# kunalchelani/EdgeGaussians

Measured on AMD Instinct MI355X. Metric: train-step Gaussians*views/sec, higher is better.
Workload: dtype f32; 1 GPU; config2: 100000 Gaussians (5:1 anisotropic, scale 0.004, opacity U(0.05,0.9)), 50 views @512x512, real poses of scan 00004926 (intrinsics 800->512); synthetic wireframe edge maps, loss whole/bg_edge_ratio 4:1; n_gaussians=100000, views=50, width=512, height=512, poses=real poses of scan 00004926 (intrinsics 800->512); synthetic wireframe edge maps, largest_tile_population=2957, gaussian_row_order=morton, binning=segmented, steps_per_native_enqueue=50, forward_mode=chained (exact transmittance stop resolved inside the forward kernel), parallelism=single GPU

## Files before the change

### edgegaussians_amd/_lib.py

```python
from __future__ import annotations

import ctypes as C
import os
from typing import Optional

import torch

_HERE = os.path.dirname(os.path.abspath(__file__))
LIB_PATH = os.path.join(_HERE, "libedgegs.so")

_vp = C.c_void_p
_i32 = C.c_int32
_i64 = C.c_int64
_u32 = C.c_uint32
_f = C.c_float

FLAG_LOG_SCALES = 1
FLAG_LOGIT_OPACITIES = 2
FLAG_ANTIALIASED = 4
FLAG_TIGHT_TILES = 8
FLAG_ABSGRAD_WRITE = 16
FLAG_FRONT_PREFIX = 32
PREFIX_HERE_MAX_TILES = 2560
REWALK_SPECULATE = -2
# ... 45 lines not shown
    "eg_tile_offsets": [_vp, _i32, _i64, _vp, _vp, _vp, _vp],
    "eg_tile_emit": [_vp, _vp, _vp, _vp, _u32, _i32, _i32, _i32, _vp, _vp, _i64, _vp, _vp, _vp],
    "eg_project_bin": [_vp] * 6 + [_i32, _i32, _i32, _u32, _vp, _vp, _vp, _i64, _vp, _vp, _vp, _vp, _vp],
    "eg_sort_pairs": [_vp, _vp, _i32, _i64, _vp, _vp, _i32, _vp],
    "eg_project_emit": [_vp] * 6 + [_i32, _i32, _i32, _u32, _vp, _vp, _i32, _vp, _vp, _i32, _vp, _vp, _vp],
    "eg_sort_segments": [_vp, _vp, _i32, _i32, _vp, _vp, _vp, _vp, _vp, _vp, _i32, _i32, _vp],
    "eg_composite_fwd_segments": [_vp] * 7 + [_i32, _i32, _vp, _vp, _vp, _vp, _vp, _f, _vp, _vp, _vp, _i64, _vp, _vp, _i32, _vp],
    "eg_composite_fwd": [_vp, _vp, _i32, _vp, _vp, _i32, _i32, _vp, _vp, _vp, _vp, _vp, _f, _vp, _vp,
                         _vp, _vp, _i64, _vp, _vp, _i32, _vp],
    "eg_composite_bwd_colors": [_vp, _vp, _i32, _vp, _vp, _i32, _i32, _vp, _vp, _vp, _vp, _vp, _vp, _vp],
    "eg_project_bwd": [_vp] * 6 + [_i32, _i32, _i32, _f, _u32] + [_vp] * 9 + [_vp],
    "eg_absgrad_accum": [_vp, _i32, _vp, _vp],
    "eg_composite_bwd_footprint": [_vp, _i32, _i32, _i32, _vp, _vp, _vp],
    "eg_backward_fused": [_vp] * 6 + [_i32, _i32, _i32, _f, _u32] + [_vp] * 10 + [C.POINTER(AdamHyper), _vp],
    "eg_adam_multi": [_vp] * 10 + [_i32, AdamHyper, _vp, _vp, _vp],
    "eg_adam_tensor": [_vp] * 4 + [_i64, C.c_double, C.c_double, C.c_double, C.c_double, _i32, _i32, _vp],
    "eg_adam_emit": [_vp] * 10 + [_i32, AdamHyper, _vp, _vp, _vp, _vp, _i32, _i32, _u32, _vp, _vp, _i32, _vp, _vp, _i32,
                     _vp, _vp, _vp],
    "eg_project_bwd_adam": [_vp] * 6 + [_i32, _i32, _i32, _f, _u32] + [_vp] * 5 + [AdamHyper, _vp],
    "eg_mask_scan": [_vp, _i32, _vp, _vp, _vp],
    "eg_compact_rows": [_vp, _vp, _vp, _i32, _i32, _vp, _vp],
    "eg_append_rows": [_vp, _vp, _vp, _i32, _i32, _i32, _i32, _vp, _f, _vp, _vp],
    "eg_ratio_wmap": [_vp, _f, _i32, _vp, _i32, _i32, _vp, _vp],
    "eg_ratio_wmap_seeded": [_vp, _f, _i32, _i32, _i32, C.c_uint64, _i32, _vp, _vp],
    "eg_ratio_wmaps_seeded": [_i32, C.POINTER(_vp), _f, C.POINTER(_i32), C.POINTER(_i32), C.POINTER(_i32), C.POINTER(C.c_uint64),
                              _i32, _vp, _vp],
    "eg_project_hits": [_vp, _i32, _vp, _i32, _vp, _i32, _i32, _vp, _vp],
    "eg_project_visibility": [_vp, _i32, _vp, _i32, _vp, _i32, _i32, _vp, _vp],
    "eg_knn": [_vp, _i32, _i32, C.POINTER(_f), _f, C.POINTER(_i32), _vp, _vp, _vp, _vp, _vp, _vp, _vp],
    "eg_knn_small": [_vp, _i32, _i32, _vp, _vp, _vp],
    "eg_knn_auto": [_vp, _i32, _i32, _vp, _vp, _vp, _vp, _vp, _vp, _vp, _vp, _f, _vp],
    "eg_nn_query_small": [_vp, _i64, _vp, _i64, _vp, _vp, _vp],
    "eg_nn_query_auto": [_vp, _i64, _vp, _i64] + [_vp] * 8 + [_vp],
    "eg_edge_sample_count": [_vp, _i32, _vp, _i32, C.c_double, _i64, _vp, _vp, _vp, _vp, _vp],
    "eg_edge_sample_emit": [_vp, _i32, _vp, _i32, _vp, _vp, _vp, _i64, _i32, _vp, _vp, _vp, _vp],
    "eg_edge_sample": [_vp, _i32, _vp, _i32, C.c_double, _i64, _i32] + [_vp] * 7 + [C.POINTER(_i32), _vp],
    "eg_direction_loss": [_vp, _vp, _vp, _vp, _i32, _i32, _i32, _vp, _vp, _vp, _vp],
    "eg_ratio_loss": [_vp, _i32, _vp, _vp, _vp],
    "eg_regulariser_step": [_i32] + [_vp] * 7 + [_i32, _vp, _i32, _i32, _i32, _i32, _vp, _f, _f, _vp, AdamHyper, _vp],
    "eg_regulariser_step_fixed": [_i32] + [_vp] * 7 + [_i32, _vp, _i32, _i32, _i32, _i32, _vp, _f, _f, _vp, AdamHyper, _vp, _vp],
    "eg_train_step": [C.POINTER(StepArgs), _vp],
    "eg_train_steps": [C.POINTER(StepArgs), _i32, C.POINTER(_i32), C.POINTER(_vp), _vp, _vp, _vp, _vp],
    "eg_train_steps_multi": [_i32, C.POINTER(C.POINTER(StepArgs)), _i32, C.POINTER(C.POINTER(_i32)), C.POINTER(C.POINTER(_vp)),
                             C.POINTER(_vp), C.POINTER(_vp), C.POINTER(_vp), C.POINTER(_vp), _i32],
    "eg_operator_fwd": [C.POINTER(OperatorArgs), _vp],
    "eg_operator_bwd": [C.POINTER(OperatorArgs), _vp, _i64, _vp, _vp, _vp, _vp, _vp, _vp, _vp, _vp, _vp],
    "eg_train_steps_dp": [C.POINTER(StepArgs), C.POINTER(AdamHyper), _vp, _i32, C.POINTER(_i32), C.POINTER(_vp), _vp, _vp,
                          _vp, _i32, _vp],
    "eg_dp_all_reduce": [_vp, _i64, _vp],
    "eg_project_fwd_cams": [_vp] * 6 + [_i32, _i32, _i32, _i32, _f, _f, _f, _f, _u32] + [_vp] * 8 + [_vp],
    "eg_project_bwd_cams": [_vp] * 6 + [_i32, _i32, _i32, _i32, _f, _u32] + [_vp] * 7 + [_vp],
    "eg_tile_offsets_cams": [_vp, _i32, _i32, _i64, _vp, _vp, _vp, _vp],
    "eg_tile_emit_sort_cams": [_vp, _vp, _vp, _i32, _i32, _i32, _i32, _vp, _vp, C.POINTER(_i64), C.POINTER(_vp), C.POINTER(_vp),
                               C.POINTER(_vp), C.POINTER(_i32), _vp],
    "eg_composite_fwd_cams": [_i32, _vp, _i32, _vp, _i32, _i32, C.POINTER(_vp), C.POINTER(_vp), _i32, _i32, _vp, _vp, _vp,
                              C.POINTER(_vp), C.POINTER(_vp), C.POINTER(_i64), C.POINTER(_vp), _vp, _vp],
    "eg_composite_bwd_footprint_cams": [_vp, _i32, _i32, _i32, _i32, _vp, _vp, _vp],
    "eg_composite_fwd_modes_cams": [_i32, _vp, _i32, _vp, _i32, _i32, _i32, _vp, _vp, _vp, _i32, _i32, _vp, _vp, _vp, _vp],
    "eg_composite_bwd_modes_cams": [_i32, _vp, _i32, _vp, _i32, _i32, _i32, _vp, _vp, _vp, _i32, _i32, _vp, _vp, _vp, _vp,
                                    _vp, _vp, _vp, _vp],
    "eg_composite_fwd_wide_cams": [_i32, _vp, _i32, _vp, _i32, _i32, _i32, _vp, _vp, _vp, _i32, _i32, _vp, _vp, _vp, _i32, _i32,
                                   _i32, _vp],
    "eg_composite_bwd_wide_cams": [_i32, _vp, _i32, _vp, _i32, _i32, _i32, _vp, _vp, _vp, _i32, _i32, _vp, _vp, _vp, _vp,
                                   _vp, _vp, _vp, _i32, _i32, _i32, _vp],
    "eg_packed_count": [_vp] * 6 + [_i32, _i32, _i32, _i32, _f, _f, _f, _f, _u32, _vp, _vp, _vp],
    "eg_packed_write": [_vp] * 6 + [_i32, _i32, _i32, _i32, _f, _f, _f, _f, _u32, _vp, _i64] + [_vp] * 10 + [_vp],
    "eg_packed_bin": [_vp, _vp, _vp, C.POINTER(_i64), _i32, _i32, _i32, _vp, _vp, C.POINTER(_i64), _vp, _vp, _vp,
                      C.POINTER(_i32), _vp],
    "eg_packed_bwd": [_vp] * 6 + [_i32, _i32, _i32, _i32, _f, _u32, _vp, _i64] + [_vp] * 7 + [_vp],
    "eg_packed_bwd_sparse": [_vp] * 6 + [_i32, _i32, _i32, _i32, _f, _u32, _i64] + [_vp] * 8 + [_vp],
    "eg_project_bwd_viewmats": [_vp] * 6 + [_i32, _i32, _i32, _i32, _f, _u32, _vp, _vp, _i64, _vp, _vp, _vp, _vp, _vp, _i32,
                                _vp, _vp],
    "eg_sh_fwd": [_i32, _i32, _i32, _i32, _vp, _vp, _vp, _vp, _i32, _vp, _i32, _vp, _vp],
    "eg_sh_bwd": [_i32, _i32, _i32, _i32, _vp, _vp, _vp, _vp, _i32, _vp, _i32, _vp, _vp, _vp, _vp, _vp],
    "eg_train_step_batched": [C.POINTER(StepArgs), _i32, C.POINTER(_vp), C.POINTER(_vp), C.POINTER(_vp), C.POINTER(_vp), _vp],
}
EXPORTS = sorted(list(_SIGS) + ["eg_last_error_string", "eg_version", "eg_device_count",
                                 "eg_composite_workspace_bytes", "eg_composite_workspace_ctl_bytes",
                                 "eg_batched_workspace_stride", "eg_knn_auto_dims", "eg_timing_begin", "eg_timing_end",
                                 "eg_timing_stage_count", "eg_timing_stage_name", "eg_debug_fwd_profile",
                                 "eg_dp_unique_id", "eg_dp_init", "eg_dp_world", "eg_dp_shutdown", "eg_dp_host_profile", "eg_roctx_enable",
                                 "eg_dp_comm_count", "eg_dp_force_all_reduce", "eg_dp_grad_all_reduces",
                                 "eg_dp_comm_timing_begin", "eg_dp_comm_timing_end", "eg_record_xcd_shift",
                                 "eg_backward_is_fused"])

_lib: Optional[C.CDLL] = None


def load(require_device: bool = True) -> C.CDLL:
    global _lib
    if _lib is None:
        if not os.path.exists(LIB_PATH):
            raise RuntimeError(
                f"{LIB_PATH} is missing: build it with `python -m edgegaussians_amd.build` "
                "(hipcc --offload-arch=gfx950).  There is no CPU fallback in the product path.")
        lib = C.CDLL(LIB_PATH)
        for name, args in _SIGS.items():
            fn = getattr(lib, name)
            fn.argtypes = args
            fn.restype = C.c_int
        lib.eg_last_error_string.restype = C.c_char_p
        lib.eg_last_error_string.argtypes = []
        lib.eg_version.restype = C.c_int
        lib.eg_device_count.restype = C.c_int
        lib.eg_timing_begin.argtypes = [_i32]
        lib.eg_timing_end.argtypes = [C.POINTER(C.c_float), C.POINTER(_i32)]
        lib.eg_timing_stage_name.argtypes = [_i32]
        lib.eg_timing_stage_name.restype = C.c_char_p
        lib.eg_composite_workspace_bytes.restype = _i64
        lib.eg_composite_workspace_bytes.argtypes = [_i64, _i64]
        lib.eg_composite_workspace_ctl_bytes.restype = _i64
        lib.eg_composite_workspace_ctl_bytes.argtypes = [_i64, _i64]
        lib.eg_batched_workspace_stride.restype = _i64
        lib.eg_batched_workspace_stride.argtypes = [_i64, _i64]
        lib.eg_knn_auto_dims.restype = _i32
        lib.eg_knn_auto_dims.argtypes = [_i32, _i32]
        lib.eg_dp_unique_id.argtypes = [C.c_char_p, _vp]
        lib.eg_dp_init.argtypes = [C.c_char_p, _vp, _i32, _i32]
        lib.eg_dp_world.argtypes = []
        lib.eg_dp_shutdown.argtypes = []
        lib.eg_roctx_enable.argtypes = [_i32]
        lib.eg_record_xcd_shift.argtypes = [_i32]
        lib.eg_backward_is_fused.argtypes = [_i32, _i32]
        lib.eg_dp_comm_count.argtypes = []
        lib.eg_dp_force_all_reduce.argtypes = [_i32]
        lib.eg_dp_grad_all_reduces.argtypes = [C.POINTER(_i64)]
        lib.eg_dp_grad_all_reduces.restype = _i64
        lib.eg_dp_comm_timing_begin.argtypes = [_i32]
        lib.eg_dp_comm_timing_end.argtypes = [C.POINTER(C.c_float), C.POINTER(C.c_float), C.POINTER(_i32)]
        lib.eg_dp_host_profile.argtypes = [C.POINTER(C.c_double)]
        lib.eg_dp_host_profile.restype = _i64
        lib.eg_debug_fwd_profile.restype = _i64
        lib.eg_debug_fwd_profile.argtypes = [_vp, _i64]
        _lib = lib
    if require_device and not torch.cuda.is_available():
        raise RuntimeError("edgegaussians_amd needs a gfx950 GPU (torch.cuda.is_available() is False); "
                           "there is no CPU fallback in the product path")
    return _lib


def composite_workspace(max_items: int, n_tiles: int, device) -> torch.Tensor:
    lib = load()
    return torch.zeros(lib.eg_composite_workspace_bytes(max_items, n_tiles), dtype=torch.uint8, device=device)


def call(name: str, *args) -> None:
    lib = load()
    rc = getattr(lib, name)(*args)
    if rc != 0:
        raise RuntimeError(f"{name} failed (code {rc}): {lib.eg_last_error_string().decode()}")


def ptr(t: Optional[torch.Tensor]) -> Optional[int]:
    if t is None:
        return None
    assert t.is_cuda and t.is_contiguous(), "libedgegs needs contiguous device tensors"
    return t.data_ptr()


_raw_stream = getattr(torch._C, "_cuda_getCurrentRawStream", None)


def stream() -> int:
    if _raw_stream is not None:
        return _raw_stream(torch.cuda.current_device())
    return torch.cuda.current_stream().cuda_stream
```

### edgegaussians_amd/csrc/binning.hip

```cpp
#include <cstdlib>

#include "common.h"
#include "composite.h"

namespace eg {

constexpr int kBinThreads = 512;
constexpr int kMaxLdsTiles = 16384;

template <bool LDS>
__global__ void __launch_bounds__(kBinThreads)
tile_count_kernel(const float2 *__restrict__ means2d, const int *__restrict__ radii, int N, int width,
                  int height, int *__restrict__ tiles_per_gauss, int *__restrict__ tile_counts) {
  extern __shared__ __attribute__((aligned(16))) int s_hist[];
  const int tw = (width + kTile - 1) / kTile, th = (height + kTile - 1) / kTile, T = tw * th;
  if (LDS) {
    for (int t = threadIdx.x; t < T; t += kBinThreads) s_hist[t] = 0;
    __syncthreads();
  }
  const int g = blockIdx.x * kBinThreads + threadIdx.x;
  if (g < N) {
    const int radius = radii[g];
    int n = 0;
    if (radius > 0) {
// ... 149 lines not shown
      if (idx < capacity) keys[idx] = key;
    }
#undef EG_TILE_OK
}


template <int THREADS>
__device__ __forceinline__ void bitonic_lds(unsigned long long *s, int P, int k_lo, int k_hi, int tid) {
  for (int k = k_lo; k <= k_hi; k <<= 1) {
    if (k <= P) {
      const int lhk = 31 - __clz(k) - 1;
      const int mk = (1 << lhk) - 1;
      for (int i = tid; i < (P >> 1); i += THREADS) {
        const int blk = i >> lhk, off = i & mk;
        const int base = blk << (lhk + 1);
        const int lo = base + off, hi = base + k - 1 - off;
        unsigned long long a = s[lo], b = s[hi];
        if (a > b) { s[lo] = b; s[hi] = a; }
      }
      __syncthreads();
    }
    for (int j = min(k >> 2, P >> 1); j >= 1; j >>= 1) {
      const int lj = 31 - __clz(j);
      for (int i = tid; i < (P >> 1); i += THREADS) {
        const int lo = ((i >> lj) << (lj + 1)) + (i & (j - 1)), hi = lo + j;
        unsigned long long a = s[lo], b = s[hi];
        if (a > b) { s[lo] = b; s[hi] = a; }
      }
      __syncthreads();
    }
  }
}

template <int THREADS>
__device__ __forceinline__ unsigned block_reduce_u32(unsigned v, bool take_max, unsigned *wave_tmp) {
  const int tid = threadIdx.x, lane = tid & 63, wv = tid >> 6;
  constexpr int NW = THREADS / 64;
#pragma unroll
  for (int d = 32; d >= 1; d >>= 1) {
    const unsigned o = __shfl_xor(v, d, 64);
    v = take_max ? max(v, o) : min(v, o);
  }
  if (lane == 0) wave_tmp[wv] = v;
  __syncthreads();
  unsigned r = wave_tmp[0];
#pragma unroll
  for (int w = 1; w < NW; ++w) r = take_max ? max(r, wave_tmp[w]) : min(r, wave_tmp[w]);
  __syncthreads();
  return r;
}

constexpr int kMaxBucketFill = 96;
constexpr int kSortBM = 2;

struct SegTable {
  int *cursor;
  int seg_cap;
  int *tile_start, *tile_end;
  int *item_first;
  int *item_end;
  int *item_tile;
  int max_items;
  int *total;
  int4 *item_rec;
  int slice_major = 0;
  const int *item_front = nullptr;
  int middle_out = 0;
  unsigned rec_tag = 0;
  int xcd_shift = 0;
  int tw = 0;
  const float *gt = nullptr, *wmap = nullptr;
  float *loss_part = nullptr;
  int width = 0, height = 0;
  int skip_empty = 0;
  float inv_tw = 0.f;
#ifdef EG_SORT_PROF
  unsigned long long *prof = nullptr;
#endif
};
constexpr int kXcdMinTiles = 512;
constexpr int kXcdShiftDefault = 1;
constexpr int kFrontDefault = 4;

template <int THREADS, int CAP, bool LARGE, bool PREFIX3 = false>
__global__ void __launch_bounds__(THREADS, THREADS == 1024 ? 1 : 4)
tile_sort_kernel(unsigned long long *__restrict__ keys, const int *__restrict__ offsets, int T,
                 long long capacity, int small_cap, int *__restrict__ flatten_ids,
                 long long *__restrict__ isect_ids, const SegTable seg_, const Batch bt) {
  extern __shared__ __attribute__((aligned(16))) unsigned long long s[];
  SegTable seg = seg_;
  {
    const int bv = blockIdx.y;
    keys += bv * bt.keys; flatten_ids += bv * bt.keys;
    if (seg.cursor) {
      seg.cursor += bv * bt.tiles; seg.tile_start += bv * bt.tiles; seg.tile_end += bv * bt.tiles;
      seg.item_first += bv * bt.tiles; seg.item_end += bv * bt.tiles; seg.item_tile += bv * bt.items;
      if (seg.total) seg.total += 4 * bv;
      if (seg.item_rec) seg.item_rec += bv * bt.items;
      if (seg.skip_empty && gridDim.y > 1) {
        seg.gt = bt.gt[bv]; seg.wmap = bt.wmap[bv];
        seg.loss_part = (float *)((char *)seg.loss_part + bv * bt.ws_bytes);
      }
    }
  }
  constexpr int BM = LARGE ? 1 : kSortBM;
  constexpr int NB = THREADS * BM;
  unsigned long long *kout = s;
  int *hist = (int *)(s + CAP);
  int *cursor = hist + NB;
  __shared__ unsigned wave_tmp[32], wave_tmp2[32];

  const int tid = threadIdx.x;
#ifdef EG_SORT_PROF
  unsigned prof_t[7] = {0u, 0u, 0u, 0u, 0u, 0u, 0u};
  const unsigned long long prof_wall0 = __builtin_amdgcn_s_memrealtime();
  long long prof_prev = (long long)__builtin_readcyclecounter();
#define EG_SP_TICK(k_)                                                           \
  do {                                                                           \
    if (!LARGE) {                                                                \
      const long long now_ = (long long)__builtin_readcyclecounter();            \
      prof_t[k_] = (unsigned)(now_ - prof_prev);                                 \
      prof_prev = now_;                                                          \
    }                                                                            \
  } while (0)
#define EG_SP_DONE(n_)                                                           \
  do {                                                                           \
    if (!LARGE && seg.prof && tid == 0 && blockIdx.y == 0) {                     \
      unsigned long long *r_ = seg.prof + (size_t)tile * 12;                     \
      r_[0] = prof_wall0; r_[1] = __builtin_amdgcn_s_memrealtime(); r_[2] = (unsigned long long)(n_); \
      r_[3] = prof_t[0]; r_[4] = prof_t[1]; r_[5] = prof_t[2]; r_[6] = prof_t[3]; r_[7] = prof_t[4]; r_[8] = prof_t[5]; r_[9] = prof_t[6]; \
      r_[10] = (unsigned long long)(__builtin_amdgcn_s_getreg(20 | (3 << 11)) & 15); r_[11] = blockIdx.x;  \
    }                                                                            \
  } while (0)
#else
#define EG_SP_TICK(k_) do {} while (0)
#define EG_SP_DONE(n_) do {} while (0)
#endif
  constexpr int kBigList = 512;
  __shared__ int s_big[LARGE ? kBigList : 1], s_big_sorted[LARGE ? kBigList : 1];
  __shared__ int s_nbig;
  int n_loop = T;
  bool by_list = false;
  if (LARGE) {
    if (tid == 0) s_nbig = 0;
    __syncthreads();
    for (int t = tid; t < T; t += THREADS) {
      long long a_, b_;
      if (seg.cursor) { a_ = seg.tile_start[t]; b_ = seg.tile_end[t]; }
      else { a_ = offsets[t]; b_ = offsets[t + 1]; if (b_ > capacity) b_ = capacity; }
      if (b_ - a_ > small_cap) {
        const int k = atomicAdd(&s_nbig, 1);
        if (k < kBigList) s_big[k] = t;
      }
    }
    __syncthreads();
    const int nb = s_nbig;
    if (nb <= kBigList) {
      for (int i = tid; i < nb; i += THREADS) {
        const int me = s_big[i];
        int rank = 0;
        for (int q = 0; q < nb; ++q) rank += s_big[q] < me ? 1 : 0;
        s_big_sorted[rank] = me;
      }
      __syncthreads();
      by_list = true;
      n_loop = nb;
    }
  }
  for (int it = blockIdx.x; it < n_loop; it += gridDim.x) {
  const int wg = by_list ? s_big_sorted[it] : it;
  const int tile = (!LARGE && seg.middle_out) ? ((wg & 1) ? T / 2 - (wg + 1) / 2 : T / 2 + wg / 2) : wg;
  __syncthreads();
  long long start, end;
  __shared__ int s_pre[5][THREADS / 64];
  bool prefix_pending = false;
  int pop_here = 0;
  auto finish_prefix = [&](int kept_) {
    prefix_pending = false;
    if (tid >= 64) return;
    int isum = 0, k0 = 0, l0k1 = 0;
#pragma unroll
    for (int w = 0; w < THREADS / 64; ++w) { isum += s_pre[0][w]; k0 += s_pre[1][w]; l0k1 += s_pre[4][w]; }
    const int first_ = min(isum, seg.max_items);
    const int items_ = min(max(1, (kept_ + 127) >> 7), max(0, seg.max_items - first_));
    const int myx = seg.xcd_shift > 0 ? xcd_of_tile(tile, seg.tw, seg.inv_tw, seg.xcd_shift) : 0;
    bool rec_over = false;
    for (int i = tid; i < items_; i += 64) {
      seg.item_tile[first_ + i] = tile;
      if (seg.item_rec) {
        const int pos = i < seg.slice_major ? k0 + i : l0k1 + (i - seg.slice_major);
        const int disp = seg.xcd_shift > 0 ? 8 * pos + myx : pos;
        if (disp >= 0 && disp < seg.max_items)
          seg.item_rec[disp] = make_int4(tile, i | (items_ << 16), (int)seg.rec_tag, tile * seg.seg_cap + kept_);
        else
          rec_over = true;
      }
    }
    if (rec_over) seg.total[1] = 1;
    if (tid == 0) {
      seg.item_first[tile] = first_;
      seg.tile_start[tile] = tile * seg.seg_cap;
      seg.tile_end[tile] = tile * seg.seg_cap + kept_;
      seg.item_end[tile] = first_ + items_;
      if (tile == T - 1) {
        int msum = 0, cmax = 0;
#pragma unroll
        for (int w = 0; w < THREADS / 64; ++w) { msum += s_pre[2][w]; cmax = max(cmax, s_pre[3][w]); }
        const int itot = isum + max(1, (kept_ + 127) >> 7);
        seg.total[0] = msum;
        if (cmax > seg.seg_cap || itot > seg.max_items) seg.total[1] = 1;
        seg.total[2] = min(itot, seg.max_items);
        seg.total[3] = cmax;
      }
    }
    prefix_pending = false;
  };
  unsigned long long spec0 = ~0ull;
  if (!LARGE && seg.cursor && tid < seg.seg_cap) spec0 = keys[(size_t)tile * seg.seg_cap + tid];
  if (seg.cursor) {
    if (!LARGE) {
      int kept, first, items;
      if (seg.total) {
        pop_here = seg.cursor[tile];
        kept = min(pop_here, seg.seg_cap);
        const __amdgpu_buffer_rsrc_t cur_rsrc = __builtin_amdgcn_make_buffer_rsrc((void *)seg.cursor, 0, T * 4, 0x00020000);
        constexpr int NE = kPrefixBatchTiles / THREADS;
        int pv0[NE];
#pragma unroll
        for (int j = 0; j < NE; ++j) pv0[j] = (int)__builtin_amdgcn_raw_buffer_load_b32(cur_rsrc, (tid + j * THREADS) * 4, 0, 0);
        constexpr bool kBgEarly = THREADS >= 512;
        auto bg_term = [&]() -> float {
          float l = 0.f;
          if (tid < kTilePix) {
            const int ty_ = (int)(((float)tile + 0.5f) * seg.inv_tw), tx_ = tile - __mul24(ty_, seg.tw);
            const int pi = ty_ * kTile + (tid >> 4), pj = tx_ * kTile + (tid & 15);
            if (pi < seg.height && pj < seg.width) {
              const int pp = pi * seg.width + pj;
              l = seg.wmap[pp] * fabsf(seg.gt[pp]);
            }
          }
          return l;
        };
        float l_bg = 0.f;
        if (kBgEarly && seg.skip_empty) l_bg = bg_term();
        if (seg.skip_empty && pop_here == 0 && tile != T - 1) {
          if (!kBgEarly) l_bg = bg_term();
          if (tid < kTilePix) {
            l_bg = wave_sum_dpp_f(l_bg);
            if ((tid & 63) == 63 && l_bg != 0.f) unsafeAtomicAdd(&seg.loss_part[(tile * 4 + (tid >> 6)) & 63], l_bg);
          }
          EG_SP_TICK(0); EG_SP_DONE(0);
          continue;
        }
        {
          int isum = 0, front = 0, deep = 0, msum = 0, cmax = 0;
          const bool last_tile = tile == T - 1;
          const int myx = seg.xcd_shift > 0 ? xcd_of_tile(tile, seg.tw, seg.inv_tw, seg.xcd_shift) : 0;
          auto sums = [&](const int (&pv)[NE], int j0) {
#pragma unroll
            for (int j = 0; j < NE; ++j) {
              const int tj = tid + (j0 + j) * THREADS;
              const bool ok = tj < T, before = tj < tile;
              const int kk = min(pv[j], seg.seg_cap), it = ok ? max(1, (kk + 127) >> 7) : 0;
              isum += before ? it : 0;
              const bool mine = (seg.xcd_shift == 0 || xcd_of_tile(tj, seg.tw, seg.inv_tw, seg.xcd_shift) == myx) &&
                                !(seg.skip_empty && kk == 0 && tj != T - 1);
              const int itf = mine ? min(it, seg.slice_major) : 0;
              front += before ? itf : 0;
              deep += itf + ((mine && before) ? it - itf : 0);
              if (last_tile) { msum += kk; cmax = max(cmax, pv[j]); }
            }
          };
          sums(pv0, 0);
          if (T > kPrefixBatchTiles) {
            int pv1[NE];
#pragma unroll
            for (int j = 0; j < NE; ++j)
              pv1[j] = (int)__builtin_amdgcn_raw_buffer_load_b32(cur_rsrc, (tid + (NE + j) * THREADS) * 4, 0, 0);
            sums(pv1, NE);
          }
          if (PREFIX3 && T > 2 * kPrefixBatchTiles) {
            int pv2[NE];
#pragma unroll
            for (int j = 0; j < NE; ++j)
              pv2[j] = (int)__builtin_amdgcn_raw_buffer_load_b32(cur_rsrc, (tid + (2 * NE + j) * THREADS) * 4, 0, 0);
            sums(pv2, 2 * NE);
          }
          isum = wave_scan_dpp(isum, 0, OpAdd());
          front = wave_scan_dpp(front, 0, OpAdd());
          deep = wave_scan_dpp(deep, 0, OpAdd());
          if (last_tile) {
            msum = wave_scan_dpp(msum, 0, OpAdd());
            cmax = wave_scan_dpp(cmax, 0, OpMaxI());
          }
          if ((tid & 63) == 63) {
            s_pre[0][tid >> 6] = isum; s_pre[1][tid >> 6] = front; s_pre[4][tid >> 6] = deep;
            if (last_tile) { s_pre[2][tid >> 6] = msum; s_pre[3][tid >> 6] = cmax; }
          }
        }
        prefix_pending = true;
        first = items = 0;
      } else {
        kept = min(seg.cursor[tile], seg.seg_cap);
        first = seg.item_first[tile];
        items = min(max(1, (kept + 127) >> 7), max(0, seg.max_items - first));
        __syncthreads();
        if (tid == 0) {
          seg.cursor[tile] = 0;
          seg.tile_start[tile] = tile * seg.seg_cap;
          seg.tile_end[tile] = tile * seg.seg_cap + kept;
          seg.item_end[tile] = first + items;
        }
        for (int i = tid; i < items; i += THREADS) {
          seg.item_tile[first + i] = tile;
          if (seg.item_rec) {
            int disp = first + i;
            if (seg.item_front) {
              const int fpre = seg.item_front[tile], ftot = seg.item_front[T];
              if (ftot >= 0) disp = i < EG_FRONT_LARGE ? fpre + i : ftot + (first - fpre) + (i - EG_FRONT_LARGE);
            }
            if (disp >= 0 && disp < seg.max_items)
              seg.item_rec[disp] = make_int4(tile, i | (items << 16), (int)seg.rec_tag, tile * seg.seg_cap + kept);
          }
        }
      }
      start = (long long)tile * seg.seg_cap;
      end = start + kept;
    } else {
      start = seg.tile_start[tile];
      end = seg.tile_end[tile];
    }
  } else {
    start = offsets[tile];
// ... 136 lines not shown
      const long long lo = blk * k + off, hi = blk * k + k - 1 - off;
      if (hi < n) {
        unsigned long long a = segk[lo], b = segk[hi];
        if (a > b) { segk[lo] = b; segk[hi] = a; }
      }
    }
    __syncthreads();
    for (long long j = k >> 2; j >= BCAP; j >>= 1) {
      for (long long i = tid; i < (P >> 1); i += THREADS) {
        const long long lo = ((i / j) * (j << 1)) + (i % j), hi = lo + j;
        if (hi < n) {
          unsigned long long a = segk[lo], b = segk[hi];
          if (a > b) { segk[lo] = b; segk[hi] = a; }
        }
      }
      __syncthreads();
    }
    for (long long c0 = 0; c0 < n; c0 += BCAP) {
      for (int i = tid; i < BCAP; i += THREADS) s[i] = (c0 + i < n) ? segk[c0 + i] : kInf;
      __syncthreads();
      bitonic_lds<THREADS>(s, BCAP, 2 * BCAP, 2 * BCAP, tid);
      for (int i = tid; i < BCAP; i += THREADS)
        if (c0 + i < n) segk[c0 + i] = s[i];
      __syncthreads();
    }
  }
  for (int i = tid; i < n; i += THREADS) {
    const unsigned long long key = segk[i];
    const int gid = (int)(unsigned)(key & 0xffffffffull);
    flatten_ids[start + i] = gid;
    if (isect_ids) isect_ids[start + i] = ((long long)tile << 32) | (long long)(key >> 32);
  }
  }
}

}

using namespace eg;

extern "C" int eg_tile_count(const float *means2d, const int32_t *radii, int32_t N, int32_t width, int32_t height,
                             int32_t *tiles_per_gauss, int32_t *tile_counts, eg_stream_t stream) {
  EG_REQUIRE(N >= 0 && width > 0 && height > 0, "bad sizes");
  if (N == 0) return EG_OK;
  EG_REQUIRE(means2d && radii && tile_counts, "null pointer");
  const int T = cdiv(width, kTile) * cdiv(height, kTile);
  if (T <= kMaxLdsTiles)
    tile_count_kernel<true><<<cdiv(N, kBinThreads), kBinThreads, sizeof(int) * T, as_stream(stream)>>>(
        (const float2 *)means2d, radii, N, width, height, tiles_per_gauss, tile_counts);
  else
    tile_count_kernel<false><<<cdiv(N, kBinThreads), kBinThreads, 0, as_stream(stream)>>>(
        (const float2 *)means2d, radii, N, width, height, tiles_per_gauss, tile_counts);
  return check_launch("tile_count");
}

extern "C" int eg_tile_offsets(const int32_t *tile_counts, int32_t T, int64_t capacity, int32_t *offsets,
                               int32_t *item_offsets, int32_t *total, eg_stream_t stream) {
  EG_REQUIRE(T > 0 && tile_counts && offsets, "bad arguments");
  tile_offsets_kernel<<<1, 1024, 0, as_stream(stream)>>>(tile_counts, T, (long long)capacity, offsets, item_offsets,
                                                        total);
  return check_launch("tile_offsets");
}

extern "C" int eg_tile_emit(const float *means2d, const int32_t *radii, const float *depths, const float *splat,
                            uint32_t flags, int32_t N, int32_t width, int32_t height, const int32_t *offsets, int32_t *tile_cursor,
                            int64_t capacity, uint64_t *keys, const uint32_t *tile_mask, eg_stream_t stream) {
  EG_REQUIRE(N >= 0 && width > 0 && height > 0 && capacity >= 0, "bad sizes");
  if (N == 0) return EG_OK;
  EG_REQUIRE(offsets && tile_cursor && (keys || capacity == 0), "null pointer");
  EG_REQUIRE(splat || (means2d && radii && depths), "need splat or (means2d, radii, depths)");
  const int T = cdiv(width, kTile) * cdiv(height, kTile);
  if (2 * T <= kMaxLdsTiles)
    tile_emit_kernel<true><<<cdiv(N, kBinThreads), kBinThreads, sizeof(int) * 2 * T, as_stream(stream)>>>(
        (const float2 *)means2d, radii, depths, (const float4 *)splat, flags, N, width, height, offsets,
        tile_cursor, (long long)capacity, (unsigned long long *)keys, tile_mask);
  else
    tile_emit_kernel<false><<<cdiv(N, kBinThreads), kBinThreads, 0, as_stream(stream)>>>(
        (const float2 *)means2d, radii, depths, (const float4 *)splat, flags, N, width, height, offsets,
        tile_cursor, (long long)capacity, (unsigned long long *)keys, tile_mask);
  return check_launch("tile_emit");
}

static bool g_sort_attr_set = false;

#ifdef EG_SORT_PROF
static unsigned long long *g_sort_prof = nullptr;
static int g_sort_prof_tiles = 0;
#endif

static int launch_tile_sort(uint64_t *keys, const int32_t *offsets, int32_t T, int64_t capacity,
                            int32_t *flatten_ids, int64_t *isect_ids, int32_t max_tile_hint, const SegTable seg_in,
                            eg_stream_t stream, const Batch &bt = Batch{}, int C = 1) {
  SegTable seg = seg_in;
#ifdef EG_SORT_PROF
  if (!g_sort_prof || g_sort_prof_tiles < T) {
    if (g_sort_prof) (void)hipFree(g_sort_prof);
    g_sort_prof_tiles = T;
    (void)hipMalloc((void **)&g_sort_prof, (size_t)T * 12 * sizeof(unsigned long long));
  }
  (void)hipMemsetAsync(g_sort_prof, 0, (size_t)T * 12 * sizeof(unsigned long long), as_stream(stream));
  seg.prof = g_sort_prof;
#endif
  constexpr int kSmall = 4096, kLarge = 16384;
  constexpr size_t kLargeLds = kLarge * 8 + 2 * 1024 * 4;
  const bool wide = max_tile_hint > 1536 && (C == 1 ? T <= 4096 : T * C <= 2048);
  if (!g_sort_attr_set) {
    (void)hipFuncSetAttribute((const void *)tile_sort_kernel<1024, kLarge, true>,
                              hipFuncAttributeMaxDynamicSharedMemorySize, (int)kLargeLds);
    g_sort_attr_set = true;
  }
  const bool small_only = max_tile_hint > 0 && (int64_t)max_tile_hint * 5 / 4 <= kSmall;
#define EG_SORT_SMALL(TH_, P3_)                                                                                          \
  tile_sort_kernel<TH_, kSmall, false, P3_><<<dim3(T, C), TH_, kSmall * 8 + 2 * TH_ * 4 * kSortBM, as_stream(stream)>>>( \
      (unsigned long long *)keys, offsets, T, (long long)capacity, small_only ? 0x7fffffff : kSmall, flatten_ids,            \
      (long long *)isect_ids, seg, bt)
  const bool prefix3 = seg.total != nullptr && T > 2 * kPrefixBatchTiles;
  if (wide) { if (prefix3) EG_SORT_SMALL(512, true); else EG_SORT_SMALL(512, false); }
  else      { if (prefix3) EG_SORT_SMALL(256, true); else EG_SORT_SMALL(256, false); }
#undef EG_SORT_SMALL
  if (!small_only)
    tile_sort_kernel<1024, kLarge, true><<<dim3(min(T, 256), C), 1024, kLargeLds, as_stream(stream)>>>(
        (unsigned long long *)keys, offsets, T, (long long)capacity, kSmall, flatten_ids, (long long *)isect_ids,
        seg, bt);
  return check_launch("tile_sort");
}

#ifdef EG_SORT_PROF
extern "C" int64_t eg_debug_sort_profile(uint64_t *out, int64_t max_tiles) {
  if (!g_sort_prof || !out) return EG_ERR_ARG;
  const int64_t n = g_sort_prof_tiles < max_tiles ? g_sort_prof_tiles : max_tiles;
  if (hipMemcpy(out, g_sort_prof, (size_t)n * 12 * sizeof(uint64_t), hipMemcpyDeviceToHost) != hipSuccess) return EG_ERR_LAUNCH;
  return n;
}
#endif

extern "C" int eg_record_xcd_shift(int32_t n_tiles) {
  return record_xcd_shift(n_tiles, n_tiles <= kPrefixHereMaxTiles, true, 1);
}

extern "C" int eg_sort_pairs(uint64_t *keys, const int32_t *offsets, int32_t T, int64_t capacity,
                             int32_t *flatten_ids, int64_t *isect_ids, int32_t max_tile_hint, eg_stream_t stream) {
  EG_REQUIRE(T > 0 && offsets, "bad arguments");
  if (capacity == 0) return EG_OK;
  EG_REQUIRE(keys && flatten_ids, "null pointer");
  return launch_tile_sort(keys, offsets, T, capacity, flatten_ids, isect_ids, max_tile_hint, SegTable{}, stream);
}

extern "C" int eg_sort_segments(uint64_t *keys, int32_t *tile_cursor, int32_t T, int32_t seg_cap,
                                int32_t *flatten_ids, int32_t *tile_start, int32_t *tile_end,
                                const int32_t *item_first, int32_t *item_end, int32_t *item_tile,
                                int32_t max_items, int32_t max_tile_hint, eg_stream_t stream) {
  EG_REQUIRE(T > 0 && seg_cap > 0 && max_items > 0, "bad sizes");
  EG_REQUIRE(keys && tile_cursor && flatten_ids && tile_start && tile_end && item_first && item_end && item_tile,
             "null pointer");
  SegTable seg;
  seg.cursor = tile_cursor; seg.seg_cap = seg_cap;
  seg.tile_start = tile_start; seg.tile_end = tile_end;
  seg.item_first = const_cast<int32_t *>(item_first); seg.item_end = item_end;
  seg.item_tile = item_tile; seg.max_items = max_items;
  seg.total = nullptr;
  seg.item_rec = nullptr;
  seg.slice_major = 0;
  return launch_tile_sort(keys, nullptr, T, (int64_t)T * seg_cap, flatten_ids, nullptr, max_tile_hint, seg, stream);
}

namespace eg {
int record_xcd_shift(int T, bool prefix_here, bool has_item_rec, int C) {
  return (prefix_here && has_item_rec && C == 1 && T >= kXcdMinTiles) ? kXcdShiftDefault : 0;
}

int launch_sort_segments(uint64_t *keys, int32_t *tile_cursor, int32_t T, int32_t seg_cap, int32_t *flatten_ids,
                         int32_t *tile_start, int32_t *tile_end, int32_t *item_first, int32_t *item_end,
                         int32_t *item_tile, int32_t max_items, int32_t max_tile_hint, const Batch &bt, int C,
                         hipStream_t st, int32_t *total_prefix_here, int32_t *item_rec, const int32_t *item_front,
                         uint32_t rec_tag, int32_t tiles_per_row, const float *gt, const float *wmap, void *workspace,
                         int32_t width, int32_t height, int32_t front_slices) {
  SegTable seg;
  seg.cursor = tile_cursor; seg.seg_cap = seg_cap;
  seg.tile_start = tile_start; seg.tile_end = tile_end;
  seg.item_first = item_first; seg.item_end = item_end;
  seg.item_tile = item_tile; seg.max_items = max_items;
  seg.total = total_prefix_here;
  seg.item_rec = (int4 *)item_rec;
  seg.slice_major = front_slices > 0 ? min(front_slices, 15) : kFrontDefault;
  seg.middle_out = 1;
  seg.item_front = total_prefix_here ? nullptr : item_front;
  seg.rec_tag = rec_tag;
  seg.tw = tiles_per_row;
  seg.inv_tw = tiles_per_row > 0 ? 1.f / (float)tiles_per_row : 0.f;
  if (total_prefix_here && item_rec && tiles_per_row > 0 && workspace && width > 0 && height > 0 &&
      (C > 1 ? bt.gt[0] && bt.wmap[0] : gt && wmap)) {
    seg.skip_empty = 1;
    seg.gt = gt; seg.wmap = wmap; seg.width = width; seg.height = height;
    seg.loss_part = carve_workspace(workspace, max_items, T).loss_part;
  }
  seg.xcd_shift = tiles_per_row > 0 ? record_xcd_shift(T, total_prefix_here != nullptr, item_rec != nullptr, C) : 0;
  return launch_tile_sort(keys, nullptr, T, (int64_t)T * seg_cap, flatten_ids, nullptr, max_tile_hint, seg,
                          (eg_stream_t)st, bt, C);
}
}
```

### include/edgegs.h

```cpp
#ifndef EDGEGS_H
#define EDGEGS_H

#include <stdint.h>

#ifdef __cplusplus
extern "C" {
#endif

typedef void *eg_stream_t;

#define EG_OK 0
#define EG_ERR_ARG (-1)
#define EG_ERR_LAUNCH (-2)
#define EG_ERR_NODEVICE (-3)
#define EG_ERR_CAPACITY (-4)

#define EG_TILE 16
#define EG_MAX_BATCH 8
#define EG_REWALK_SPECULATE (-2)
#define EG_FLAG_LOG_SCALES 1u
#define EG_FLAG_LOGIT_OPACITIES 2u
#define EG_FLAG_ANTIALIASED 4u
#define EG_FLAG_ABSGRAD_WRITE 16u
#define EG_FLAG_FRONT_PREFIX 32u
// ... 162 lines not shown
int eg_nn_query_small(const float *queries , int64_t Q, const float *targets , int64_t M,
                      int32_t *out_idx , float *out_d2 , eg_stream_t stream);
int eg_nn_query_auto(const float *queries , int64_t Q, const float *targets , int64_t M,
                     int32_t *cell_of, int32_t *cell_counts, int32_t *cell_start, float *sorted_targets,
                     float *sorted_queries, void *grid_scratch, int32_t *out_idx , float *out_d2 ,
                     eg_stream_t stream);
int eg_edge_sample_count(const double *curves , int32_t Nc, const double *lines , int32_t Nl,
                         double resolution , int64_t capacity, double *lengths ,
                         int32_t *counts , int32_t *offsets , int32_t *total ,
                         eg_stream_t stream);
#define EG_EDGE_TANGENT_REFERENCE 0
#define EG_EDGE_TANGENT_EXACT 1
int eg_edge_sample_emit(const double *curves, int32_t Nc, const double *lines, int32_t Nl,
                        const int32_t *counts , const int32_t *offsets ,
                        const int32_t *total , int64_t capacity, int32_t tangent, float *points ,
                        float *directions , int32_t *prim_ids ,
                        eg_stream_t stream);
int eg_edge_sample(const double *curves, int32_t Nc, const double *lines, int32_t Nl, double resolution,
                   int64_t capacity, int32_t tangent, double *lengths, int32_t *counts, int32_t *offsets,
                   int32_t *total , float *points, float *directions, int32_t *prim_ids,
                   int32_t *total_host , eg_stream_t stream);
int eg_direction_loss(const float *means, const float *quats, const float *log_scales,
                      const int32_t *nn_idx , int32_t N, int32_t K, int32_t top_k,
                      float *g_means , float *g_quats , float *sum_out,
                      eg_stream_t stream);
int eg_ratio_loss(const float *log_scales, int32_t N, float *g_scales , float *sum_out,
                  eg_stream_t stream);

int eg_regulariser_step(int32_t kind, float *means, float *quats, float *log_scales, float *logit_opacities,
                        float *adam_m, float *adam_v, float *grads, int32_t N, const int32_t *nn, int32_t nn_stride,
                        int32_t nn_offset, int32_t K, int32_t top_k, const float *loss_sum, float loss_sum_host,
                        float scale_factor, float *work , eg_adam_hyper hyper, eg_stream_t stream);
int eg_regulariser_step_fixed(int32_t kind, float *means, float *quats, float *log_scales, float *logit_opacities,
                              float *adam_m, float *adam_v, float *grads, int32_t N, const int32_t *nn, int32_t nn_stride,
                              int32_t nn_offset, int32_t K, int32_t top_k, const float *loss_sum, float loss_sum_host,
                              float scale_factor, float *work , eg_adam_hyper hyper, int64_t *fixed ,
                              eg_stream_t stream);

int eg_ratio_wmap(const float *gt , float thr, int32_t n_edge, const int64_t *perm, int32_t n_sel, int32_t HW,
                  float *out , eg_stream_t stream);

int eg_ratio_wmap_seeded(const float *gt , float thr, int32_t n_edge, int32_t n_bg, int32_t n_sel,
                         uint64_t seed, int32_t HW, float *out , eg_stream_t stream);
int eg_ratio_wmaps_seeded(int32_t C, const float *const *gts, float thr, const int32_t *n_edge, const int32_t *n_bg,
                          const int32_t *n_sel, const uint64_t *seeds, int32_t HW, float *out , eg_stream_t stream);

typedef struct {
  float *means, *quats, *log_scales, *logit_opacities;
  float *adam_m, *adam_v, *absgrads;
  int32_t N;
  const float *viewmat, *K, *gt, *wmap;
  int32_t width, height;
  float loss_scale;
  float *splat, *g2d;
  int32_t *tile_counts, *offsets, *item_offsets, *total;
  uint32_t *tile_mask;
  int32_t *ticket;
  void *workspace;
  int64_t max_items;
  uint64_t *keys;
  int32_t *flatten_ids;
  int64_t capacity;
  int32_t max_tile_hint;
  int32_t rewalk_hint;
  int32_t seg_cap;
  int32_t *tile_end, *item_end, *item_tile;
  float *render, *alphas, *vpix, *loss;
  float *gtstop;
  int32_t *last_ids;
  float *v_means, *v_quats, *v_scales, *v_opacities;
  const eg_adam_hyper *adam_host;
  const float *next_viewmat, *next_K;
  int32_t have_projection;
  int32_t ws_tag;
  int32_t *item_rec;
  int32_t two_kernel_backward;
} eg_step_args;
#define EG_MAX_WS_TAG 0xfffe

int eg_train_step(const eg_step_args *args_host, eg_stream_t stream);

int eg_backward_is_fused(int32_t n_gaussians, int32_t n_tiles);

int eg_record_xcd_shift(int32_t n_tiles);

int eg_train_steps(const eg_step_args *args_host, int32_t K, const int32_t *views_host,
                   const float *const *wmaps_host, const float *viewmats, const float *Ks, const float *gts,
                   eg_stream_t stream);

int eg_train_steps_multi(int32_t S, const eg_step_args *const *args_host, int32_t K, const int32_t *const *views_host,
                         const float *const *const *wmaps_host, const float *const *viewmats, const float *const *Ks,
                         const float *const *gts, const eg_stream_t *streams, int32_t n_threads);

int64_t eg_batched_workspace_stride(int64_t max_items, int64_t n_tiles);
int eg_train_step_batched(const eg_step_args *args_host, int32_t C, const float *const *viewmats,
                          const float *const *Ks, const float *const *gts, const float *const *wmaps,
                          eg_stream_t stream);

int eg_project_fwd_cams(const float *means, const float *quats, const float *scales, const float *opacities,
                        const float *viewmats , const float *Ks , int32_t N, int32_t C, int32_t width,
                        int32_t height, float near_plane, float far_plane, float eps2d, float radius_clip, uint32_t flags,
                        float *splat , int32_t *radii, float *means2d, float *depths, float *conics,
                        float *compensations, int32_t *tiles_per_gauss ,
                        int32_t *tile_counts , eg_stream_t stream);
int eg_project_bwd_cams(const float *means, const float *quats, const float *scales, const float *opacities,
                        const float *viewmats, const float *Ks, int32_t N, int32_t C, int32_t width, int32_t height, float eps2d,
                        uint32_t flags, const float *splat , const float *g2d ,
                        const float *v_comps_ext , const float *v_depths_ext , float *v_means,
                        float *v_quats, float *v_scales, eg_stream_t stream);
int eg_tile_offsets_cams(const int32_t *tile_counts , int32_t T, int32_t C, int64_t capacity,
                         int32_t *offsets , int32_t *item_offsets , int32_t *total ,
                         eg_stream_t stream);
int eg_tile_emit_sort_cams(const float *means2d , const int32_t *radii , const float *depths ,
                           int32_t N, int32_t C, int32_t width, int32_t height, const int32_t *offsets ,
                           int32_t *tile_counts , const int64_t *M_host ,
                           uint64_t *const *keys, int32_t *const *flatten_ids, int64_t *const *isect_ids ,
                           const int32_t *max_tile_host , eg_stream_t stream);
int eg_composite_fwd_cams(int32_t C, const float *splat , int32_t N, const float *colors, int32_t colors_per_camera,
                          int32_t channels, const int32_t *const *offsets, const int32_t *const *flatten_ids, int32_t width,
                          int32_t height, float *render , float *alphas ,
                          int32_t *last_ids , const int32_t *const *item_offsets, const int32_t *const *total,
                          const int64_t *max_items_host, void *const *workspace, float *gtstop ,
                          eg_stream_t stream);
int eg_composite_bwd_footprint_cams(const float *splat , int32_t N, int32_t C, int32_t width, int32_t height,
                                    const float *gtstop , float *g2d , eg_stream_t stream);

int eg_composite_fwd_modes_cams(int32_t C, const float *splat , int32_t N, const float *colors,
                                int32_t colors_per_camera, int32_t channels, int32_t depth,
                                const float *backgrounds , const int32_t *offsets ,
                                const int32_t *flatten_ids, int32_t width, int32_t height, float *render, float *alphas,
                                int32_t *last_ids, eg_stream_t stream);
int eg_composite_bwd_modes_cams(int32_t C, const float *splat , int32_t N, const float *colors,
                                int32_t colors_per_camera, int32_t channels, int32_t depth,
                                const float *backgrounds , const int32_t *offsets ,
                                const int32_t *flatten_ids, int32_t width, int32_t height, const float *alphas,
                                const int32_t *last_ids, const float *v_render, const float *v_alphas ,
                                float *g2d , float *v_colors ,
                                float *v_depths , eg_stream_t stream);

int eg_composite_fwd_wide_cams(int32_t C, const float *splat , int32_t N, const float *colors,
                               int32_t colors_per_camera, int32_t channels, int32_t depth,
                               const float *backgrounds , const int32_t *offsets ,
                               const int32_t *flatten_ids, int32_t width, int32_t height, float *render,
                               float *alphas , int32_t *last_ids , int32_t n_real,
                               int32_t color_stride, int32_t pixel_stride, eg_stream_t stream);
int eg_composite_bwd_wide_cams(int32_t C, const float *splat , int32_t N, const float *colors,
                               int32_t colors_per_camera, int32_t channels, int32_t depth,
                               const float *backgrounds , const int32_t *offsets ,
                               const int32_t *flatten_ids, int32_t width, int32_t height, const float *alphas,
                               const int32_t *last_ids, const float *v_render, const float *v_alphas ,
                               float *g2d , float *v_colors , float *v_depths ,
                               int32_t n_real, int32_t color_stride, int32_t pixel_stride, eg_stream_t stream);

#define EG_PACKED_STRIDE 0

int eg_packed_count(const float *means, const float *quats, const float *scales, const float *opacities,
                    const float *viewmats , const float *Ks , int32_t N, int32_t C, int32_t width,
                    int32_t height, float near_plane, float far_plane, float eps2d, float radius_clip, uint32_t flags,
                    int32_t *block_base , int64_t *indptr , eg_stream_t stream);
int eg_packed_write(const float *means, const float *quats, const float *scales, const float *opacities,
                    const float *viewmats, const float *Ks, int32_t N, int32_t C, int32_t width, int32_t height,
                    float near_plane, float far_plane, float eps2d, float radius_clip, uint32_t flags,
                    const int32_t *block_base, int64_t nnz, float *splat , int32_t *radii, float *means2d,
                    float *depths, float *conics, float *compensations, int32_t *tiles_per_gauss, int64_t *camera_ids,
                    int64_t *gaussian_ids, int32_t *tile_counts , eg_stream_t stream);
int eg_packed_bin(const float *means2d , const int32_t *radii , const float *depths ,
// ... 83 lines not shown
```

Measured before the change: 1.285 billion Gaussians*views/s.

## Sort two tiles per workgroup with shared prefix scan in tile sort

Adds a paired mode to the tile sort kernel where each workgroup processes tile rank r and its mirror T-1-r, halving the grid. Both tiles' cursor prefix sums are computed in one pass over the cursor array, and their speculative keys are preloaded together. Empty tiles contribute background loss without taking a sort pass. This is meant to cut redundant prefix scans and balance heavy and light tiles within one workgroup, at the cost of serialising two tile sorts per workgroup and using more registers and shared memory.

```diff
diff --git a/edgegaussians_amd/_lib.py b/edgegaussians_amd/_lib.py
--- a/edgegaussians_amd/_lib.py
+++ b/edgegaussians_amd/_lib.py
@@ -151,7 +151,7 @@
                                  "eg_dp_unique_id", "eg_dp_init", "eg_dp_world", "eg_dp_shutdown", "eg_dp_host_profile", "eg_roctx_enable",
                                  "eg_dp_comm_count", "eg_dp_force_all_reduce", "eg_dp_grad_all_reduces",
                                  "eg_dp_comm_timing_begin", "eg_dp_comm_timing_end", "eg_record_xcd_shift",
-                                 "eg_backward_is_fused"])
+                                 "eg_backward_is_fused", "eg_sort_two_tiles_per_workgroup"])
 
 _lib: Optional[C.CDLL] = None
 
@@ -191,6 +191,7 @@
         lib.eg_roctx_enable.argtypes = [_i32]
         lib.eg_record_xcd_shift.argtypes = [_i32]
         lib.eg_backward_is_fused.argtypes = [_i32, _i32]
+        lib.eg_sort_two_tiles_per_workgroup.argtypes = [_i32, _i32]
         lib.eg_dp_comm_count.argtypes = []
         lib.eg_dp_force_all_reduce.argtypes = [_i32]
         lib.eg_dp_grad_all_reduces.argtypes = [C.POINTER(_i64)]
diff --git a/edgegaussians_amd/csrc/binning.hip b/edgegaussians_amd/csrc/binning.hip
--- a/edgegaussians_amd/csrc/binning.hip
+++ b/edgegaussians_amd/csrc/binning.hip
@@ -255,7 +255,26 @@
 constexpr int kXcdShiftDefault = 1;
 constexpr int kFrontDefault = 4;
 
-template <int THREADS, int CAP, bool LARGE, bool PREFIX3 = false>
+__device__ __forceinline__ float bg_loss_term(const SegTable &seg, int tile, int tid) {
+  float l = 0.f;
+  if (tid < kTilePix) {
+    const int ty_ = (int)(((float)tile + 0.5f) * seg.inv_tw), tx_ = tile - __mul24(ty_, seg.tw);
+    const int pi = ty_ * kTile + (tid >> 4), pj = tx_ * kTile + (tid & 15);
+    if (pi < seg.height && pj < seg.width) {
+      const int pp = pi * seg.width + pj;
+      l = seg.wmap[pp] * fabsf(seg.gt[pp]);
+    }
+  }
+  return l;
+}
+__device__ __forceinline__ void add_bg_loss(const SegTable &seg, int tile, int tid, float l_bg) {
+  if (tid < kTilePix) {
+    l_bg = wave_sum_dpp_f(l_bg);
+    if ((tid & 63) == 63 && l_bg != 0.f) unsafeAtomicAdd(&seg.loss_part[(tile * 4 + (tid >> 6)) & 63], l_bg);
+  }
+}
+
+template <int THREADS, int CAP, bool LARGE, bool PREFIX3 = false, bool PAIR = false>
 __global__ void __launch_bounds__(THREADS, THREADS == 1024 ? 1 : 4)
 tile_sort_kernel(unsigned long long *__restrict__ keys, const int *__restrict__ offsets, int T,
                  long long capacity, int small_cap, int *__restrict__ flatten_ids,
@@ -305,9 +324,24 @@
       r_[10] = (unsigned long long)(__builtin_amdgcn_s_getreg(20 | (3 << 11)) & 15); r_[11] = blockIdx.x;  \
     }                                                                            \
   } while (0)
+#define EG_SP_NEXT()                                                             \
+  do {                                                                           \
+    if (PAIR && pass > 0) {                                                      \
+      for (int k_ = 0; k_ < 7; ++k_) prof_t[k_] = 0u;                            \
+      prof_prev = (long long)__builtin_readcyclecounter();                       \
+    }                                                                            \
+  } while (0)
+#define EG_SP_EMPTY()                                                            \
+  do {                                                                           \
+    prof_t[0] = (unsigned)((long long)__builtin_readcyclecounter() - prof_prev); \
+    EG_SP_DONE(0);                                                               \
+    prof_t[0] = 0u;                                                              \
+  } while (0)
 #else
 #define EG_SP_TICK(k_) do {} while (0)
 #define EG_SP_DONE(n_) do {} while (0)
+#define EG_SP_NEXT() do {} while (0)
+#define EG_SP_EMPTY() do {} while (0)
 #endif
   constexpr int kBigList = 512;
   __shared__ int s_big[LARGE ? kBigList : 1], s_big_sorted[LARGE ? kBigList : 1];
@@ -340,12 +374,110 @@
       n_loop = nb;
     }
   }
-  for (int it = blockIdx.x; it < n_loop; it += gridDim.x) {
+  __shared__ int s_pre[PAIR ? 10 : 5][THREADS / 64];
+  int tileA = 0, tileB = 0, popA = 0, popB = 0, n_pass = 0;
+  bool goA = false;
+  unsigned long long specA = ~0ull, specB = ~0ull;
+  if (PAIR) {
+    const int rA = blockIdx.x, rB = T - 1 - rA;
+    const bool hasB = rB != rA;
+    auto tile_of_rank = [&](int r) { return seg.middle_out ? ((r & 1) ? T / 2 - (r + 1) / 2 : T / 2 + r / 2) : r; };
+    tileA = tile_of_rank(rA);
+    tileB = hasB ? tile_of_rank(rB) : tileA;
+    if (tid < seg.seg_cap) {
+      specA = keys[(size_t)tileA * seg.seg_cap + tid];
+      if (hasB) specB = keys[(size_t)tileB * seg.seg_cap + tid];
+    }
+    popA = seg.cursor[tileA];
+    popB = seg.cursor[tileB];
+    const __amdgpu_buffer_rsrc_t cur_rsrc = __builtin_amdgcn_make_buffer_rsrc((void *)seg.cursor, 0, T * 4, 0x00020000);
+    constexpr int NE = kPrefixBatchTiles / THREADS;
+    static_assert(!(PAIR && PREFIX3), "pairs are launched on grids of <= 2 prefix batches (launch_tile_sort)");
+    int pv0[NE], pv1[NE];
+#pragma unroll
+    for (int j = 0; j < NE; ++j) {
+      pv0[j] = (int)__builtin_amdgcn_raw_buffer_load_b32(cur_rsrc, (tid + j * THREADS) * 4, 0, 0);
+      pv1[j] = 0;
+    }
+    if (T > kPrefixBatchTiles) {
+#pragma unroll
+      for (int j = 0; j < NE; ++j)
+        pv1[j] = (int)__builtin_amdgcn_raw_buffer_load_b32(cur_rsrc, (tid + (NE + j) * THREADS) * 4, 0, 0);
+    }
+    float lA = 0.f, lB = 0.f;
+    if (seg.skip_empty) {
+      lA = bg_loss_term(seg, tileA, tid);
+      if (hasB) lB = bg_loss_term(seg, tileB, tid);
+    }
+    const bool emptyA = seg.skip_empty && popA == 0 && tileA != T - 1;
+    const bool emptyB = hasB && seg.skip_empty && popB == 0 && tileB != T - 1;
+    goA = !emptyA;
+    const bool goB = hasB && !emptyB;
+    n_pass = (goA ? 1 : 0) + (goB ? 1 : 0);
+    if (n_pass > 0) {
+      int isA = 0, frA = 0, dpA = 0, isB = 0, frB = 0, dpB = 0, msum = 0, cmax = 0;
+      const bool any_last = tileA == T - 1 || tileB == T - 1;
+      const int xA = seg.xcd_shift > 0 ? xcd_of_tile(tileA, seg.tw, seg.inv_tw, seg.xcd_shift) : 0;
+      const int xB = seg.xcd_shift > 0 ? xcd_of_tile(tileB, seg.tw, seg.inv_tw, seg.xcd_shift) : 0;
+      auto sums2 = [&](const int (&pv)[NE], int j0) {
+#pragma unroll
+        for (int j = 0; j < NE; ++j) {
+          const int tj = tid + (j0 + j) * THREADS;
+          const bool ok = tj < T, beforeA = tj < tileA, beforeB = tj < tileB;
+          const int kk = min(pv[j], seg.seg_cap), it = ok ? max(1, (kk + 127) >> 7) : 0;
+          const bool rec = !(seg.skip_empty && kk == 0 && tj != T - 1);
+          const int xj = seg.xcd_shift > 0 ? xcd_of_tile(tj, seg.tw, seg.inv_tw, seg.xcd_shift) : 0;
+          const int itf = rec ? min(it, seg.slice_major) : 0, itd = rec ? it - itf : 0;
+          const int itfA = xj == xA ? itf : 0, itfB = xj == xB ? itf : 0;
+          isA += beforeA ? it : 0;
+          frA += beforeA ? itfA : 0;
+          dpA += itfA + ((xj == xA && beforeA) ? itd : 0);
+          isB += beforeB ? it : 0;
+          frB += beforeB ? itfB : 0;
+          dpB += itfB + ((xj == xB && beforeB) ? itd : 0);
+          if (any_last) { msum += kk; cmax = max(cmax, pv[j]); }
+        }
+      };
+      sums2(pv0, 0);
+      if (T > kPrefixBatchTiles) sums2(pv1, NE);
+      const bool top = (tid & 63) == 63;
+      if (goA) {
+        isA = wave_scan_dpp(isA, 0, OpAdd());
+        frA = wave_scan_dpp(frA, 0, OpAdd());
+        dpA = wave_scan_dpp(dpA, 0, OpAdd());
+        if (top) { s_pre[0][tid >> 6] = isA; s_pre[1][tid >> 6] = frA; s_pre[4][tid >> 6] = dpA; }
+      }
+      if (goB) {
+        isB = wave_scan_dpp(isB, 0, OpAdd());
+        frB = wave_scan_dpp(frB, 0, OpAdd());
+        dpB = wave_scan_dpp(dpB, 0, OpAdd());
+        if (top) { s_pre[5][tid >> 6] = isB; s_pre[6][tid >> 6] = frB; s_pre[9][tid >> 6] = dpB; }
+      }
+      if (any_last) {
+        msum = wave_scan_dpp(msum, 0, OpAdd());
+        cmax = wave_scan_dpp(cmax, 0, OpMaxI());
+        const int lb = tileA == T - 1 ? 0 : 5;
+        if (top) { s_pre[lb + 2][tid >> 6] = msum; s_pre[lb + 3][tid >> 6] = cmax; }
+      }
+    }
+    if (emptyA) {
+      add_bg_loss(seg, tileA, tid, lA);
+      { const int tile = tileA; (void)tile; EG_SP_EMPTY(); }
+    }
+    if (emptyB) {
+      add_bg_loss(seg, tileB, tid, lB);
+      { const int tile = tileB; (void)tile; EG_SP_EMPTY(); }
+    }
+  }
+  for (int it = blockIdx.x, pass = 0; PAIR ? pass < n_pass : it < n_loop; it += gridDim.x, ++pass) {
+  const bool useB = PAIR && (pass > 0 || !goA);
   const int wg = by_list ? s_big_sorted[it] : it;
-  const int tile = (!LARGE && seg.middle_out) ? ((wg & 1) ? T / 2 - (wg + 1) / 2 : T / 2 + wg / 2) : wg;
-  __syncthreads();
+  const int tile = PAIR ? (useB ? tileB : tileA)
+                        : (!LARGE && seg.middle_out) ? ((wg & 1) ? T / 2 - (wg + 1) / 2 : T / 2 + wg / 2) : wg;
+  if (!PAIR || pass > 0) __syncthreads();
+  EG_SP_NEXT();
   long long start, end;
-  __shared__ int s_pre[5][THREADS / 64];
+  const int pb = (PAIR && useB) ? 5 : 0;
   bool prefix_pending = false;
   int pop_here = 0;
   auto finish_prefix = [&](int kept_) {
@@ -353,7 +485,7 @@
     if (tid >= 64) return;
     int isum = 0, k0 = 0, l0k1 = 0;
 #pragma unroll
-    for (int w = 0; w < THREADS / 64; ++w) { isum += s_pre[0][w]; k0 += s_pre[1][w]; l0k1 += s_pre[4][w]; }
+    for (int w = 0; w < THREADS / 64; ++w) { isum += s_pre[pb + 0][w]; k0 += s_pre[pb + 1][w]; l0k1 += s_pre[pb + 4][w]; }
     const int first_ = min(isum, seg.max_items);
     const int items_ = min(max(1, (kept_ + 127) >> 7), max(0, seg.max_items - first_));
     const int myx = seg.xcd_shift > 0 ? xcd_of_tile(tile, seg.tw, seg.inv_tw, seg.xcd_shift) : 0;
@@ -378,7 +510,7 @@
       if (tile == T - 1) {
         int msum = 0, cmax = 0;
 #pragma unroll
-        for (int w = 0; w < THREADS / 64; ++w) { msum += s_pre[2][w]; cmax = max(cmax, s_pre[3][w]); }
+        for (int w = 0; w < THREADS / 64; ++w) { msum += s_pre[pb + 2][w]; cmax = max(cmax, s_pre[pb + 3][w]); }
         const int itot = isum + max(1, (kept_ + 127) >> 7);
         seg.total[0] = msum;
         if (cmax > seg.seg_cap || itot > seg.max_items) seg.total[1] = 1;
@@ -389,11 +521,17 @@
     prefix_pending = false;
   };
   unsigned long long spec0 = ~0ull;
-  if (!LARGE && seg.cursor && tid < seg.seg_cap) spec0 = keys[(size_t)tile * seg.seg_cap + tid];
+  if (PAIR) spec0 = useB ? specB : specA;
+  else if (!LARGE && seg.cursor && tid < seg.seg_cap) spec0 = keys[(size_t)tile * seg.seg_cap + tid];
   if (seg.cursor) {
     if (!LARGE) {
       int kept, first, items;
-      if (seg.total) {
+      if (PAIR) {
+        pop_here = useB ? popB : popA;
+        kept = min(pop_here, seg.seg_cap);
+        prefix_pending = true;
+        first = items = 0;
+      } else if (seg.total) {
         pop_here = seg.cursor[tile];
         kept = min(pop_here, seg.seg_cap);
         const __amdgpu_buffer_rsrc_t cur_rsrc = __builtin_amdgcn_make_buffer_rsrc((void *)seg.cursor, 0, T * 4, 0x00020000);
@@ -402,26 +540,12 @@
 #pragma unroll
         for (int j = 0; j < NE; ++j) pv0[j] = (int)__builtin_amdgcn_raw_buffer_load_b32(cur_rsrc, (tid + j * THREADS) * 4, 0, 0);
         constexpr bool kBgEarly = THREADS >= 512;
-        auto bg_term = [&]() -> float {
-          float l = 0.f;
-          if (tid < kTilePix) {
-            const int ty_ = (int)(((float)tile + 0.5f) * seg.inv_tw), tx_ = tile - __mul24(ty_, seg.tw);
-            const int pi = ty_ * kTile + (tid >> 4), pj = tx_ * kTile + (tid & 15);
-            if (pi < seg.height && pj < seg.width) {
-              const int pp = pi * seg.width + pj;
-              l = seg.wmap[pp] * fabsf(seg.gt[pp]);
-            }
-          }
-          return l;
-        };
+        auto bg_term = [&]() -> float { return bg_loss_term(seg, tile, tid); };
         float l_bg = 0.f;
         if (kBgEarly && seg.skip_empty) l_bg = bg_term();
         if (seg.skip_empty && pop_here == 0 && tile != T - 1) {
           if (!kBgEarly) l_bg = bg_term();
-          if (tid < kTilePix) {
-            l_bg = wave_sum_dpp_f(l_bg);
-            if ((tid & 63) == 63 && l_bg != 0.f) unsafeAtomicAdd(&seg.loss_part[(tile * 4 + (tid >> 6)) & 63], l_bg);
-          }
+          add_bg_loss(seg, tile, tid, l_bg);
           EG_SP_TICK(0); EG_SP_DONE(0);
           continue;
         }
@@ -724,6 +848,11 @@
 
 static bool g_sort_attr_set = false;
 
+extern "C" int eg_sort_two_tiles_per_workgroup(int32_t n_tiles, int32_t max_tile_hint) {
+  constexpr int kResident = 512;
+  return (max_tile_hint > 1536 && n_tiles > kResident && n_tiles <= 2 * kPrefixBatchTiles) ? 1 : 0;
+}
+
 #ifdef EG_SORT_PROF
 static unsigned long long *g_sort_prof = nullptr;
 static int g_sort_prof_tiles = 0;
@@ -751,13 +880,16 @@
     g_sort_attr_set = true;
   }
   const bool small_only = max_tile_hint > 0 && (int64_t)max_tile_hint * 5 / 4 <= kSmall;
-#define EG_SORT_SMALL(TH_, P3_)                                                                                          \
-  tile_sort_kernel<TH_, kSmall, false, P3_><<<dim3(T, C), TH_, kSmall * 8 + 2 * TH_ * 4 * kSortBM, as_stream(stream)>>>( \
+  const bool pair = seg.total != nullptr && C == 1 && eg_sort_two_tiles_per_workgroup(T, max_tile_hint) != 0;
+#define EG_SORT_SMALL(TH_, P3_, PR_)                                                                                     \
+  tile_sort_kernel<TH_, kSmall, false, P3_, PR_><<<dim3(PR_ ? (T + 1) / 2 : T, C), TH_, kSmall * 8 + 2 * TH_ * 4 * kSortBM, \
+                                                   as_stream(stream)>>>(                                                 \
       (unsigned long long *)keys, offsets, T, (long long)capacity, small_only ? 0x7fffffff : kSmall, flatten_ids,            \
       (long long *)isect_ids, seg, bt)
   const bool prefix3 = seg.total != nullptr && T > 2 * kPrefixBatchTiles;
-  if (wide) { if (prefix3) EG_SORT_SMALL(512, true); else EG_SORT_SMALL(512, false); }
-  else      { if (prefix3) EG_SORT_SMALL(256, true); else EG_SORT_SMALL(256, false); }
+  if (pair)      { EG_SORT_SMALL(512, false, true); }
+  else if (wide) { if (prefix3) EG_SORT_SMALL(512, true, false); else EG_SORT_SMALL(512, false, false); }
+  else           { if (prefix3) EG_SORT_SMALL(256, true, false); else EG_SORT_SMALL(256, false, false); }
 #undef EG_SORT_SMALL
   if (!small_only)
     tile_sort_kernel<1024, kLarge, true><<<dim3(min(T, 256), C), 1024, kLargeLds, as_stream(stream)>>>(
diff --git a/include/edgegs.h b/include/edgegs.h
--- a/include/edgegs.h
+++ b/include/edgegs.h
@@ -268,6 +268,8 @@
 
 int eg_backward_is_fused(int32_t n_gaussians, int32_t n_tiles);
 
+int eg_sort_two_tiles_per_workgroup(int32_t n_tiles, int32_t max_tile_hint);
+
 int eg_record_xcd_shift(int32_t n_tiles);
 
 int eg_train_steps(const eg_step_args *args_host, int32_t K, const int32_t *views_host,
```

Result: faster. 1.300 billion Gaussians*views/s (median of 6 runs) (+1.2%).
